# LMP88959/Digital-Subband-Video-1

Hardware: AMD Instinct MI355X
Metric: encoded Mpixels/sec, 1080p 4:2:0 GOP=12, bit-exact .dsv (higher is better)
Workload: dtype u8/int16+int32 (bit-exact; packed int16 inside a proven range, int32 escape)

## Files before the change

digital-subband-video-1_amd/csrc/k_sbt.hip:

```cpp
#include <type_traits>
#include "dsvg_dev.hpp"
#include <algorithm>
#include "dsvg_kernels.hpp"
#include "dsvg_host.hpp"

template <int M>
static __device__ __forceinline__ void store_row(int32_t *p, const int (&v)[M], int n)
{
    if (n >= M) {
        if (M == 4 && (((uintptr_t)p) & 15) == 0) {
            *reinterpret_cast<int4 *>(p) = make_int4(v[0], v[1 % M], v[2 % M], v[3 % M]);
            return;
        }
        if (M == 2 && (((uintptr_t)p) & 7) == 0) {
            *reinterpret_cast<int2 *>(p) = make_int2(v[0], v[1 % M]);
            return;
        }
#pragma unroll
        for (int i = 0; i < M; i++) p[i] = v[i];
    } else {
#pragma unroll
        for (int i = 0; i < M; i++)
            if (i < n) p[i] = v[i];
    }
// ... 358 lines not shown
static __device__ __forceinline__ s16x2 pk_rdiv2(s16x2 v) { return (v + (short)1 + (v >> 15)) >> 1; }
static __device__ __forceinline__ s16x2 pk_rdiv4(s16x2 v) { return (v + (short)2 + (v >> 15)) >> 2; }
static __device__ __forceinline__ s16x2 pk_div4(s16x2 v) { return (v + ((v >> 15) & (short)3)) >> 2; }
struct PkRow { s16x2 e0, e1, o0, o1; };
static __device__ __forceinline__ s16x2 pk_u(unsigned v) { return __builtin_bit_cast(s16x2, v); }
static __device__ __forceinline__ unsigned pk_b(s16x2 v) { return __builtin_bit_cast(unsigned, v); }
#define PK_EVEN(hi_, lo_) pk_u((lo_) & 0x00ff00ffu)
#define PK_ODD(hi_, lo_) pk_u(__builtin_amdgcn_perm(0u, (lo_), 0x0c030c01u))
#define PK_E2(hi_, lo_) pk_u(__builtin_amdgcn_perm((hi_), (lo_), 0x0c040c02u))
#define PK_O2(hi_, lo_) pk_u(__builtin_amdgcn_perm((hi_), (lo_), 0x0c050c03u))
static __device__ __forceinline__ PkRow pk_unpack8(unsigned lo, unsigned hi)
{
    return PkRow{PK_EVEN(0u, lo), PK_EVEN(0u, hi), PK_ODD(0u, lo), PK_ODD(0u, hi)};
}
static __device__ __forceinline__ void pk_bytes8(const PkRow &p, unsigned &lo, unsigned &hi)
{
    lo = (pk_b(p.o0) << 8) | pk_b(p.e0);
    hi = (pk_b(p.o1) << 8) | pk_b(p.e1);
}
template <typename EMITPK>
static __device__ __forceinline__ void mc_luma_patch_hpk(const DSVG_GLOBAL uint8_t *gr, int stride, bool xh, EMITPK emit_pk)
{
    const unsigned shb = (unsigned)(((uintptr_t)gr) & 3);
    const DSVG_GLOBAL uint8_t *ga = gr - shb;
    U4A4 rw[8];
#pragma unroll
    for (int r = 0; r < 8; r++) { const dsvg_u32x4a4 t = *reinterpret_cast<const DSVG_GLOBAL dsvg_u32x4a4 *>(ga + (r + 1) * stride); rw[r] = U4A4{t.x, t.y, t.z, t.w}; }
    __builtin_amdgcn_sched_barrier(0);
    const s16x2 z = s16x2{0, 0}, m255 = s16x2{255, 255};
    auto H = [&](s16x2 a, s16x2 b, s16x2 c, s16x2 d) {
        const s16x2 t = ((b + c) * (short)9 + (short)8 - (a + d)) >> 4;
        const s16x2 u = pk_min(pk_max(t, z), m255);
        return xh ? u : b;
    };
#pragma unroll
    for (int r = 0; r < 8; r++) {
        const unsigned lo = __builtin_amdgcn_alignbyte(rw[r].y, rw[r].x, shb), mi = __builtin_amdgcn_alignbyte(rw[r].z, rw[r].y, shb),
                       hi = __builtin_amdgcn_alignbyte(rw[r].w, rw[r].z, shb);
        const s16x2 A0 = PK_EVEN(0u, lo), A1 = PK_ODD(0u, lo), A2 = PK_E2(mi, lo), A3 = PK_O2(mi, lo), A4 = PK_EVEN(0u, mi), A5 = PK_ODD(0u, mi),
                    A6 = PK_E2(hi, mi), A7 = PK_O2(hi, mi), A8 = PK_EVEN(0u, hi);
        emit_pk(r, PkRow{H(A0, A1, A2, A3), H(A4, A5, A6, A7), H(A1, A2, A3, A4), H(A5, A6, A7, A8)});
    }
}

#define MCB(lo, mi, hi, m) ((int)((((m) < 4 ? (lo) : ((m) < 8 ? (mi) : (hi))) >> (8 * ((m) & 3))) & 0xff))
static __device__ __forceinline__ void mc_pack8(const int (&pv)[8], unsigned &plo, unsigned &phi)
{
    plo = (unsigned)pv[0] | ((unsigned)pv[1] << 8) | ((unsigned)pv[2] << 16) | ((unsigned)pv[3] << 24);
    phi = (unsigned)pv[4] | ((unsigned)pv[5] << 8) | ((unsigned)pv[6] << 16) | ((unsigned)pv[7] << 24);
}
struct NoEmitInts {};
template <bool AX, bool AY, typename EMIT, typename EMITI = NoEmitInts>
static __device__ __forceinline__ void mc_luma_patch(const DSVG_GLOBAL uint8_t *gr, int stride, bool xh, bool yh, EMIT emit, EMITI emit_i = EMITI{})
{
    auto out8 = [&](int r, const int (&pv)[8]) {
        if constexpr (std::is_same_v<EMITI, NoEmitInts>) {
            unsigned pl, ph_;
            mc_pack8(pv, pl, ph_);
            emit(r, pl, ph_);
        } else {
            emit_i(r, pv);
        }
    };
    const unsigned shb = (unsigned)(((uintptr_t)gr) & 3);
    const DSVG_GLOBAL uint8_t *ga = gr - shb;
    if (!AY) {
        U4A4 rw[8];
#pragma unroll
        for (int r = 0; r < 8; r++) { const dsvg_u32x4a4 t = *reinterpret_cast<const DSVG_GLOBAL dsvg_u32x4a4 *>(ga + (r + 1) * stride); rw[r] = U4A4{t.x, t.y, t.z, t.w}; }
        __builtin_amdgcn_sched_barrier(0);
#pragma unroll
        for (int r = 0; r < 8; r++) {
            const unsigned lo = __builtin_amdgcn_alignbyte(rw[r].y, rw[r].x, shb), mi = __builtin_amdgcn_alignbyte(rw[r].z, rw[r].y, shb),
                           hi = __builtin_amdgcn_alignbyte(rw[r].w, rw[r].z, shb);
            if (!AX) {
                emit(r, __builtin_amdgcn_alignbyte(mi, lo, 1u), __builtin_amdgcn_alignbyte(hi, mi, 1u));
            } else {
                int bq[11], pv[8];
#pragma unroll
                for (int m = 0; m < 11; m++) bq[m] = MCB(lo, mi, hi, m);
#pragma unroll
                for (int i = 0; i < 8; i++) {
                    const int t = (9 * (bq[i + 1] + bq[i + 2]) - (bq[i] + bq[i + 3]) + 8) >> 4;
                    pv[i] = xh ? d_sat8(t) : bq[i + 1];
                }
                out8(r, pv);
            }
        }
    } else {
        U4A4 rw[11];
#pragma unroll
        for (int k = 0; k < 11; k++) { const dsvg_u32x4a4 t = *reinterpret_cast<const DSVG_GLOBAL dsvg_u32x4a4 *>(ga + k * stride); rw[k] = U4A4{t.x, t.y, t.z, t.w}; }
        __builtin_amdgcn_sched_barrier(0);
        int Hq[4][8];
#pragma unroll
        for (int k = 0; k < 11; k++) {
            const unsigned lo = __builtin_amdgcn_alignbyte(rw[k].y, rw[k].x, shb), mi = __builtin_amdgcn_alignbyte(rw[k].z, rw[k].y, shb),
                           hi = __builtin_amdgcn_alignbyte(rw[k].w, rw[k].z, shb);
            int bq[11];
#pragma unroll
            for (int m = 0; m < 11; m++) bq[m] = MCB(lo, mi, hi, m);
#pragma unroll
            for (int i = 0; i < 8; i++) Hq[k & 3][i] = (AX && xh) ? 9 * (bq[i + 1] + bq[i + 2]) - (bq[i] + bq[i + 3]) : 16 * bq[i + 1];
            if (k >= 3) {
                const int r = k - 3;
                int pv[8];
#pragma unroll
                for (int i = 0; i < 8; i++) {
                    const int h0 = Hq[r & 3][i], h1 = Hq[(r + 1) & 3][i], h2 = Hq[(r + 2) & 3][i], h3 = Hq[(r + 3) & 3][i];
                    const int v = yh ? 9 * (h1 + h2) - (h0 + h3) : 16 * h1;
                    pv[i] = d_sat8((v + 128) >> 8);
                }
                out8(r, pv);
            }
        }
    }
}
template <bool AX, typename EMITPK>
static __device__ __forceinline__ void mc_luma_patch_vpk(const DSVG_GLOBAL uint8_t *gr, int stride, bool xh, bool yh, EMITPK emit_pk)
{
    const unsigned shb = (unsigned)(((uintptr_t)gr) & 3);
    const DSVG_GLOBAL uint8_t *ga = gr - shb;
    U4A4 rw[11];
#pragma unroll
    for (int k = 0; k < 11; k++) { const dsvg_u32x4a4 t = *reinterpret_cast<const DSVG_GLOBAL dsvg_u32x4a4 *>(ga + k * stride); rw[k] = U4A4{t.x, t.y, t.z, t.w}; }
    __builtin_amdgcn_sched_barrier(0);
    auto Hrow = [&](s16x2 a, s16x2 b, s16x2 c, s16x2 d) {
        const s16x2 g = b << 4;
        if (!AX) return g;
        const s16x2 f = (b + c) * (short)9 - (a + d);
        return xh ? f : g;
    };
    auto V = [&](s16x2 a0, s16x2 a1, s16x2 a2, s16x2 a3) {
        const s16x2 u = a1 + (yh ? a2 : a1), w = (yh ? a0 : a1) + (yh ? a3 : a1);
        const int vx = (9 * (int)u.x - (int)w.x + 128) >> 8, vy = (9 * (int)u.y - (int)w.y + 128) >> 8;
        return pk2(d_sat8(vx), d_sat8(vy));
    };
    PkRow Hq[4];
#pragma unroll
    for (int k = 0; k < 11; k++) {
        const unsigned lo = __builtin_amdgcn_alignbyte(rw[k].y, rw[k].x, shb), mi = __builtin_amdgcn_alignbyte(rw[k].z, rw[k].y, shb),
                       hi = __builtin_amdgcn_alignbyte(rw[k].w, rw[k].z, shb);
        const s16x2 A0 = PK_EVEN(0u, lo), A1 = PK_ODD(0u, lo), A2 = PK_E2(mi, lo), A3 = PK_O2(mi, lo), A4 = PK_EVEN(0u, mi), A5 = PK_ODD(0u, mi),
                    A6 = PK_E2(hi, mi), A7 = PK_O2(hi, mi), A8 = PK_EVEN(0u, hi);
        Hq[k & 3] = PkRow{Hrow(A0, A1, A2, A3), Hrow(A4, A5, A6, A7), Hrow(A1, A2, A3, A4), Hrow(A5, A6, A7, A8)};
        if (k >= 3) {
            const int r = k - 3;
            const PkRow &h0 = Hq[r & 3], &h1 = Hq[(r + 1) & 3], &h2 = Hq[(r + 2) & 3], &h3 = Hq[(r + 3) & 3];
            emit_pk(r, PkRow{V(h0.e0, h1.e0, h2.e0, h3.e0), V(h0.e1, h1.e1, h2.e1, h3.e1), V(h0.o0, h1.o0, h2.o0, h3.o0), V(h0.o1, h1.o1, h2.o1, h3.o1)});
        }
    }
}
struct __attribute__((aligned(4))) U3A4 { unsigned x, y, z; };
template <bool ANY, typename EMIT>
static __device__ __forceinline__ void mc_chroma_patch(const DSVG_GLOBAL uint8_t *gr, int stride, bool xh, bool yh, EMIT emit)
{
    const DSVG_GLOBAL uint8_t *g1 = gr + 1;
    const unsigned shb = (unsigned)(((uintptr_t)g1) & 3);
    const DSVG_GLOBAL uint8_t *ga = g1 - shb;
    constexpr int NR = ANY ? 9 : 8;
    U3A4 rw[NR];
#pragma unroll
    for (int k = 0; k < NR; k++) { const dsvg_u32x3a4 t = *reinterpret_cast<const DSVG_GLOBAL dsvg_u32x3a4 *>(ga + (k + 1) * stride); rw[k] = U3A4{t.x, t.y, t.z}; }
    __builtin_amdgcn_sched_barrier(0);
    unsigned qlo = 0, qhi = 0, qx = 0;
#pragma unroll
    for (int k = 0; k < NR; k++) {
        const unsigned lo = __builtin_amdgcn_alignbyte(rw[k].y, rw[k].x, shb), hi = __builtin_amdgcn_alignbyte(rw[k].z, rw[k].y, shb),
                       x8 = rw[k].z >> (8 * shb);
        if (!ANY) {
            emit(k, lo, hi);
        } else if (k >= 1) {
            int pv[8];
#pragma unroll
            for (int i = 0; i < 8; i++) {
                const int pa = MCB(qlo, qhi, qx, i), pb = MCB(qlo, qhi, qx, i + 1), pc = MCB(lo, hi, x8, i), pd = MCB(lo, hi, x8, i + 1);
                const int B = xh ? pb : pa, C = yh ? pc : pa, D = xh ? (yh ? pd : pb) : (yh ? pc : pa);
                pv[i] = (pa + B + C + D + 2) >> 2;
            }
            unsigned pl, ph_;
            mc_pack8(pv, pl, ph_);
            emit(k - 1, pl, ph_);
        }
        qlo = lo; qhi = hi; qx = x8;
    }
}

template <typename EMITPK>
static __device__ __forceinline__ void mc_chroma_patch_pk(const DSVG_GLOBAL uint8_t *gr, int stride, bool xh, bool yh, EMITPK emit_pk)
{
    const DSVG_GLOBAL uint8_t *g1 = gr + 1;
    const unsigned shb = (unsigned)(((uintptr_t)g1) & 3);
    const DSVG_GLOBAL uint8_t *ga = g1 - shb;
    U3A4 rw[9];
#pragma unroll
    for (int k = 0; k < 9; k++) { const dsvg_u32x3a4 t = *reinterpret_cast<const DSVG_GLOBAL dsvg_u32x3a4 *>(ga + (k + 1) * stride); rw[k] = U3A4{t.x, t.y, t.z}; }
    __builtin_amdgcn_sched_barrier(0);
    const s16x2 two = s16x2{2, 2};
    PkRow hp;
#pragma unroll
    for (int k = 0; k < 9; k++) {
        const unsigned lo = __builtin_amdgcn_alignbyte(rw[k].y, rw[k].x, shb), hi = __builtin_amdgcn_alignbyte(rw[k].z, rw[k].y, shb),
                       x8 = rw[k].z >> (8 * shb);
        const s16x2 A0 = PK_EVEN(0u, lo), A1 = PK_ODD(0u, lo), A2 = PK_E2(hi, lo), A4 = PK_EVEN(0u, hi), A5 = PK_ODD(0u, hi), A6 = PK_E2(x8, hi);
        const PkRow h = PkRow{A0 + (xh ? A1 : A0), A4 + (xh ? A5 : A4), A1 + (xh ? A2 : A1), A5 + (xh ? A6 : A5)};
        if (k >= 1)
            emit_pk(k - 1, PkRow{(hp.e0 + (yh ? h.e0 : hp.e0) + two) >> 2, (hp.e1 + (yh ? h.e1 : hp.e1) + two) >> 2,
                                 (hp.o0 + (yh ? h.o0 : hp.o0) + two) >> 2, (hp.o1 + (yh ? h.o1 : hp.o1) + two) >> 2});
        hp = h;
    }
}

struct FwdFastQ {
    int sh1[4];
    int q2[2], q3;
    float rc2[2], rc3;
};
static __device__ __forceinline__ int sym_shift(int v, int sh) { return (v + ((v >> 31) & ((1 << sh) - 1))) >> sh; }
static __device__ __forceinline__ void put_row4(const QCtx &q, int pos, s16x2 ab, s16x2 cd)
{
    const unsigned x = __builtin_bit_cast(unsigned, ab), y = __builtin_bit_cast(unsigned, cd);
    if (!(x | y)) return;
#ifndef FWD_FAST_NO_ROW4
    if ((pos & 3) == 0) {
        typedef unsigned row4_t __attribute__((ext_vector_type(2)));
        row4_t v;
        v.x = x; v.y = y;
        *reinterpret_cast<DSVG_GLOBAL row4_t *>(q.sym + pos) = v;
        q.nzf[pos >> 2] = 1;
        q.cfl[pos >> 11] = 1;
        return;
    }
#endif
    if (ab.x) q.put_sparse(pos, ab.x);
    if (ab.y) q.put_sparse(pos + 1, ab.y);
    if (cd.x) q.put_sparse(pos + 2, cd.x);
    if (cd.y) q.put_sparse(pos + 3, cd.y);
}
static __device__ __forceinline__ void put_row4(const QCtx &q, int pos, int a, int b, int c, int d)
{
    if (!(a | b | c | d)) return;
#ifndef FWD_FAST_NO_ROW4
    if ((pos & 3) == 0) {
        typedef unsigned row4_t __attribute__((ext_vector_type(2)));
        row4_t v;
        v.x = ((unsigned)a & 0xffffu) | ((unsigned)b << 16);
        v.y = ((unsigned)c & 0xffffu) | ((unsigned)d << 16);
        *reinterpret_cast<DSVG_GLOBAL row4_t *>(q.sym + pos) = v;
        q.nzf[pos >> 2] = 1;
        q.cfl[pos >> 11] = 1;
        return;
    }
#endif
    if (a) q.put_sparse(pos, a);
    if (b) q.put_sparse(pos + 1, b);
    if (c) q.put_sparse(pos + 2, c);
    if (d) q.put_sparse(pos + 3, d);
}

static __device__ __forceinline__ void fwd_fast_rows1(const QCtx &q, const QLevel &L1, int sh1, int cx1, int cy1,
                                                      const int (&r0)[8], const int (&r1)[8], int (&out)[4])
{
    int mx = max(r0[0], r0[1]), mn = min(r0[0], r0[1]);
#pragma unroll
    for (int i = 2; i < 8; i += 2) { mx = max(mx, max(r0[i], r0[i + 1])); mn = min(mn, min(r0[i], r0[i + 1])); }
#pragma unroll
    for (int i = 0; i < 8; i += 2) { mx = max(mx, max(r1[i], r1[i + 1])); mn = min(mn, min(r1[i], r1[i + 1])); }
    if (4 * max(mx, -mn) < (1 << sh1)) {
#pragma unroll
        for (int i = 0; i < 4; i++) out[i] = (r0[2 * i] + r0[2 * i + 1]) + (r1[2 * i] + r1[2 * i + 1]);
        return;
    }
    int slh[4], shl[4], shh[4], any = 0;
#pragma unroll
    for (int i = 0; i < 4; i++) {
        const int s0 = r0[2 * i] + r0[2 * i + 1], s1 = r1[2 * i] + r1[2 * i + 1];
        const int d0 = r0[2 * i] - r0[2 * i + 1], d1 = r1[2 * i] - r1[2 * i + 1];
        out[i] = s0 + s1;
        slh[i] = sym_shift(d0 + d1, sh1); shl[i] = sym_shift(s0 - s1, sh1); shh[i] = sym_shift(d0 - d1, sh1);
        any |= slh[i] | shl[i] | shh[i];
    }
    if (any) {
        q.nz_any = 1;
        const int pr = cy1 * L1.sw + cx1;
        put_row4(q, L1.base0 + pr, slh[0], slh[1], slh[2], slh[3]);
        put_row4(q, L1.base1 + pr, shl[0], shl[1], shl[2], shl[3]);
        put_row4(q, L1.base2 + pr, shh[0], shh[1], shh[2], shh[3]);
    }
}
static __device__ __forceinline__ void fwd_fast_rows1_pk(const QCtx &q, const QLevel &L1, int sh1, int cx1, int cy1,
                                                         const PkRow &r0, const PkRow &r1, int (&out)[4])
{
    const s16x2 s0a = r0.e0 + r0.o0, s0b = r0.e1 + r0.o1, d0a = r0.e0 - r0.o0, d0b = r0.e1 - r0.o1;
    const s16x2 s1a = r1.e0 + r1.o0, s1b = r1.e1 + r1.o1, d1a = r1.e0 - r1.o0, d1b = r1.e1 - r1.o1;
    const s16x2 lla = s0a + s1a, llb = s0b + s1b;
    const s16x2 lha = d0a + d1a, lhb = d0b + d1b, hla = s0a - s1a, hlb = s0b - s1b, hha = d0a - d1a, hhb = d0b - d1b;
    out[0] = lla.x; out[1] = lla.y; out[2] = llb.x; out[3] = llb.y;
    const s16x2 mx = pk_max(pk_max(pk_max(lha, lhb), pk_max(hla, hlb)), pk_max(hha, hhb));
    const s16x2 mn = pk_min(pk_min(pk_min(lha, lhb), pk_min(hla, hlb)), pk_min(hha, hhb));
    const s16x2 am = pk_max(mx, s16x2{0, 0} - mn);
    if ((pk_b(am) & ~(((1u << min(sh1, 15)) - 1u) * 0x00010001u)) == 0) return;
    q.nz_any = 1;
    const int pr = cy1 * L1.sw + cx1;
    const short ms = (short)((1 << sh1) - 1), ss = (short)sh1;
    const s16x2 mm = {ms, ms}, sv = {ss, ss}, s15 = {15, 15};
    auto pks = [&](s16x2 v) { return (v + ((v >> s15) & mm)) >> sv; };
    put_row4(q, L1.base0 + pr, pks(lha), pks(lhb));
    put_row4(q, L1.base1 + pr, pks(hla), pks(hlb));
    put_row4(q, L1.base2 + pr, pks(hha), pks(hhb));
}
template <int N, int HZL>
static __device__ __forceinline__ void fwd_fast_level(const QCtx &q, const QLevel &L, const int (&qqv)[N / 2], const float (&rcv)[N / 2], int cx0, int cy0,
                                                      const int (&in)[N][N], int (&out)[N / 2][N / 2])
{
#pragma unroll
    for (int j = 0; j < N / 2; j++)
#pragma unroll
        for (int i = 0; i < N / 2; i++) {
            const int qq = qqv[j];
            const float rc = rcv[j];
            const int a = in[2 * j][2 * i], b = in[2 * j][2 * i + 1], c = in[2 * j + 1][2 * i], d = in[2 * j + 1][2 * i + 1];
            const int s0 = a + b, s1 = c + d, d0 = a - b, d1 = c - d;
            out[j][i] = d_ll_down(s0 + s1);
            const int vlh = d0 + d1, vhl = s0 - s1, vhh = d0 - d1;
#ifndef FWD_FAST_NO_QTEST
            if (max(max(max(vlh, vhl), vhh), -min(min(vlh, vhl), vhh)) < qq) continue;
#endif
            int slh, shl, shh;
            (void)q_coef<HZL>(qq, rc, vlh, slh);
            (void)q_coef<HZL>(qq, rc, vhl, shl);
            (void)q_coef<HZL>(qq, rc, vhh, shh);
            if (slh | shl | shh) {
                q.nz_any = 1;
                const int pr = (cy0 + j) * L.sw + cx0 + i;
                if (slh) q.put_sparse(L.base0 + pr, slh);
                if (shl) q.put_sparse(L.base1 + pr, shl);
                if (shh) q.put_sparse(L.base2 + pr, shh);
            }
        }
}

#ifndef FWD_FAST_INTRA
#define FWD_FAST_INTRA 1
#endif
struct FwdFastSel { bool ok, intra; QLevel L1, L2, L3; int i1[4], i2[2], i3; };
struct FwdFastHp { QLevel L1, L2, L3; int nbh; bool ovx, ovy, sparse; };
static __device__ __forceinline__ FwdFastHp fwd_fast_hp(const JobDev &jb, const HzPlane &hp)
{
    FwdFastHp H;
    const int sw0 = hp.s_w[0], sw1 = hp.s_w[1], sw2 = hp.s_w[2], sh0 = hp.s_h[0], sh1 = hp.s_h[1], sh2 = hp.s_h[2];
    H.L1 = q_level<2>(hp); H.L2 = q_level<1>(hp); H.L3 = q_level<0>(hp);
    H.nbh = hp.nbh;
    H.ovx = (int)(2 * sw0 > sw1) | (int)(2 * sw1 > sw2);
    H.ovy = (int)(2 * sh0 > sh1) | (int)(2 * sh1 > sh2);
    H.sparse = jb.nzf != nullptr;
    return H;
}
static __device__ __forceinline__ FwdFastSel fwd_fast_sel(const FwdFastHp &H, int mode, int I, int J, int x0, int y0, int pw, int ph)
{
    FwdFastSel S;
    S.ok = false; S.intra = mode != 0;
    if (H.sparse && (FWD_FAST_INTRA || mode == 0) && x0 + 8 <= pw && y0 + 8 <= ph && !(H.ovx && I == 0) && !(H.ovy && J == 0)) {
        S.L1 = H.L1; S.L2 = H.L2; S.L3 = H.L3;
        const int nbh = H.nbh;
        const int b1x = (4 * I * S.L1.dbx) >> 14, b2x = (2 * I * S.L2.dbx) >> 14;
        S.ok = b1x == ((4 * I + 3) * S.L1.dbx) >> 14 && b2x == ((2 * I + 1) * S.L2.dbx) >> 14;
#pragma unroll
        for (int j = 0; j < 4; j++) S.i1[j] = (((4 * J + j) * S.L1.dby) >> 14) * nbh + b1x;
#pragma unroll
        for (int j = 0; j < 2; j++) S.i2[j] = (((2 * J + j) * S.L2.dby) >> 14) * nbh + b2x;
        S.i3 = ((J * S.L3.dby) >> 14) * nbh + ((I * S.L3.dbx) >> 14);
    }
    return S;
}
static __device__ __forceinline__ FwdFastSel fwd_fast_sel(const JobDev &jb, const HzPlane &hp, bool any_ov, int mode, int I, int J,
                                                          int x0, int y0, int pw, int ph)
{
    (void)any_ov;
    return fwd_fast_sel(fwd_fast_hp(jb, hp), mode, I, J, x0, y0, pw, ph);
}

template <int CH>
static __device__ __forceinline__ void fwd_mc_fast_body(const JobDev *__restrict__ jobs, const SbtGeo3 &G, const McGeo &MG, int c0, int npl,
                                                        const DMV *__restrict__ mvs0, XcdGrid XG, int plain)
{
    Blk3 B;
    if (!d_xcd_blk3(XG, B, plain != 0)) return;
    int job, c;
    d_job_plane(B.z, npl, c0, job, c);
    const SbtGeo g = G.g[c];
    const int I = B.x * 64 + threadIdx.x, J = B.y * 4 + threadIdx.y;
    if (I >= g.w3 || J >= g.h3) return;
    const JobDev &jb = jobs[job];
    const int sh = CH ? MG.hs : 0, sv = CH ? MG.vs : 0;
    const int bw = MG.blk_w >> sh, bh = MG.blk_h >> sv;
    const int pw = MG.w[c], ph = g.ph, stride = g.pstride;
    const int x0 = 8 * I, y0 = 8 * J;
    const int bi = (int)(((float)I + 0.5f) * __builtin_amdgcn_rcpf((float)(bw >> 3)));
    const int bj = (int)(((float)J + 0.5f) * __builtin_amdgcn_rcpf((float)(bh >> 3)));
    const int nblk = MG.nbh * MG.nbv, blk = bj * MG.nbh + bi;
    const HzPlane &hp = jb.hz[c];
    FwdFastHp H = fwd_fast_hp(jb, hp);
    const DMV *mvtab = jb.mvs;
    const uint8_t *stable_p = jb.stable, *srcp_p = jb.srcp[c];
    int sstride = jb.srcs[c];
#define FWD_PIN(x) asm volatile("" : "+s"(x))
#ifndef FWD_FAST_NO_PIN
    FWD_PIN(H.L1.sh0); FWD_PIN(H.L1.sh1); FWD_PIN(H.L1.dbx); FWD_PIN(H.L1.dby); FWD_PIN(H.L2.qp); FWD_PIN(H.L2.dbx); FWD_PIN(H.L2.dby);
    FWD_PIN(H.L3.qp); FWD_PIN(H.L3.dbx); FWD_PIN(H.L3.dby); FWD_PIN(H.nbh); FWD_PIN(mvtab); FWD_PIN(stable_p); FWD_PIN(srcp_p); FWD_PIN(sstride);
#endif
    DMV mv;
    {
        const auto mq = reinterpret_cast<const DSVG_GLOBAL char *>(dsvg_global(mvs0 ? mvs0 + (size_t)job * nblk : mvtab)) + (unsigned)blk * (unsigned)sizeof(DMV);
        const unsigned xy = *reinterpret_cast<const DSVG_GLOBAL unsigned *>(mq);
        mv.x = (int16_t)(xy & 0xffffu); mv.y = (int16_t)(xy >> 16); mv.mode = *reinterpret_cast<const DSVG_GLOBAL uint8_t *>(mq + 4);
    }
    QCtx q;
    q.hp = &hp; q.stable = dsvg_global(stable_p);
    q.sym = dsvg_global(jb.sym + jb.nz_off[c]);
    q.any_ov = H.ovx | H.ovy;
    q.nzf = H.sparse ? dsvg_global(jb.nzf + (jb.nz_off[c] >> 2)) : nullptr;
    q.cfl = H.sparse ? dsvg_global(jb.cflag + jb.chunk_off[c]) : nullptr;
    const FwdFastSel S = fwd_fast_sel(H, mv.mode, I, J, x0, y0, pw, ph);
    if (!S.ok) return;
    const QLevel &L1 = S.L1, &L2 = S.L2, &L3 = S.L3;
    const auto sp = dsvg_global(srcp_p);
    uint2 sw[8];
    if (S.intra) {
        const auto px = dsvg_global(static_cast<const uint8_t *>(jb.xf + g.poff));
#pragma unroll
        for (int r = 0; r < 8; r++) sw[r] = dsvg_ld2(px + (unsigned)((y0 + r) * stride + x0));
    } else {
#pragma unroll
        for (int r = 0; r < 8; r++) sw[r] = dsvg_ld2(sp + (unsigned)((y0 + r) * sstride + x0));
    }
    int f1[4], f2[2];
#pragma unroll
    for (int j = 0; j < 4; j++) f1[j] = q.stable[S.i1[j]];
#pragma unroll
    for (int j = 0; j < 2; j++) f2[j] = q.stable[S.i2[j]];
    const int f3 = q.stable[S.i3];
    FwdFastQ fq;
    const int dx = mv.x >> sh, dy = mv.y >> sv;
    const int xb = bi * bw, yb = bj * bh;
    const int wx = d_clamp(xb + (dx >> 1), -DSVG_BORDER, pw - bw + DSVG_BORDER - 1) + (x0 - xb);
    const int wy = d_clamp(yb + (dy >> 1), -DSVG_BORDER, ph - bh + DSVG_BORDER - 1) + (y0 - yb);
    const bool xh = !S.intra && (dx & 1), yh = !S.intra && (dy & 1);
    const auto gr = dsvg_global(static_cast<const uint8_t *>(jb.ref + g.poff)) + ((wy - 1) * stride + (wx - 1));
    const bool any_x = __ballot(xh) != 0ull, any_y = __ballot(yh) != 0ull;
    const auto pp = dsvg_global(jb.pred + g.poff);
#ifndef FWD_FAST_NO_PK
    int l1[4][4];
    PkRow rp[2];
    const s16x2 cmin = s16x2{-128, -128}, cmax = s16x2{127, 127};
    auto emit_core = [&](int r, const PkRow &P, unsigned plo, unsigned phi) {
        const PkRow Sr = pk_unpack8(sw[r].x, sw[r].y);
        PkRow &R = rp[r & 1];
        R.e0 = pk_min(pk_max(Sr.e0 - P.e0, cmin), cmax); R.e1 = pk_min(pk_max(Sr.e1 - P.e1, cmin), cmax);
        R.o0 = pk_min(pk_max(Sr.o0 - P.o0, cmin), cmax); R.o1 = pk_min(pk_max(Sr.o1 - P.o1, cmin), cmax);
        dsvg_st2(pp + (unsigned)((y0 + r) * stride + x0), make_uint2(plo, phi));
        if (r & 1) fwd_fast_rows1_pk(q, L1, f1[r >> 1] ? L1.sh1 : L1.sh0, 4 * I, 4 * J + (r >> 1), rp[0], rp[1], l1[r >> 1]);
    };
    auto emit = [&](int r, unsigned plo, unsigned phi) { emit_core(r, pk_unpack8(plo, phi), plo, phi); };
    auto emit_pk = [&](int r, const PkRow &P) {
        unsigned plo, phi;
        pk_bytes8(P, plo, phi);
        emit_core(r, P, plo, phi);
    };
    if (S.intra) {
        const s16x2 c128 = s16x2{128, 128};
#pragma unroll
        for (int r = 0; r < 8; r++) {
            const PkRow X = pk_unpack8(sw[r].x, sw[r].y);
            PkRow &R = rp[r & 1];
            R.e0 = X.e0 - c128; R.e1 = X.e1 - c128; R.o0 = X.o0 - c128; R.o1 = X.o1 - c128;
            if (r & 1) fwd_fast_rows1_pk(q, L1, f1[r >> 1] ? L1.sh1 : L1.sh0, 4 * I, 4 * J + (r >> 1), rp[0], rp[1], l1[r >> 1]);
        }
    } else
#ifdef FWD_FAST_NO_VPK
    auto emit_i = [&](int r, const int (&pv)[8]) { emit_pk(r, PkRow{pk2(pv[0], pv[2]), pk2(pv[4], pv[6]), pk2(pv[1], pv[3]), pk2(pv[5], pv[7])}); };
#endif
    if (CH == 0) {
#ifdef FWD_FAST_NO_VPK
        if (any_y) mc_luma_patch<true, true>(gr, stride, xh, yh, emit, emit_i);
#else
        if (any_y && any_x) mc_luma_patch_vpk<true>(gr, stride, xh, yh, emit_pk);
        else if (any_y) mc_luma_patch_vpk<false>(gr, stride, xh, yh, emit_pk);
#endif
        else if (any_x) mc_luma_patch_hpk(gr, stride, xh, emit_pk);
        else mc_luma_patch<false, false>(gr, stride, xh, yh, emit);
    } else {
        if (any_x || any_y) mc_chroma_patch_pk(gr, stride, xh, yh, emit_pk);
        else mc_chroma_patch<false>(gr, stride, xh, yh, emit);
    }
#else
    int l1[4][4], ra[2][8];
    auto emit = [&](int r, unsigned plo, unsigned phi) {
        int (&row)[8] = ra[r & 1];
#pragma unroll
        for (int i = 0; i < 8; i++) {
            const int sv_ = (int)(((i < 4 ? sw[r].x : sw[r].y) >> (8 * (i & 3))) & 0xff);
            const int pv_ = (int)(((i < 4 ? plo : phi) >> (8 * (i & 3))) & 0xff);
            row[i] = d_clamp(sv_ - pv_, -128, 127);
        }
        dsvg_st2(pp + (unsigned)((y0 + r) * stride + x0), make_uint2(plo, phi));
        if (r & 1) fwd_fast_rows1(q, L1, f1[r >> 1] ? L1.sh1 : L1.sh0, 4 * I, 4 * J + (r >> 1), ra[0], ra[1], l1[r >> 1]);
    };
    if (CH == 0) {
        if (any_y) mc_luma_patch<true, true>(gr, stride, xh, yh, emit);
        else if (any_x) mc_luma_patch<true, false>(gr, stride, xh, yh, emit);
        else mc_luma_patch<false, false>(gr, stride, xh, yh, emit);
    } else {
        if (any_x || any_y) mc_chroma_patch<true>(gr, stride, xh, yh, emit);
        else mc_chroma_patch<false>(gr, stride, xh, yh, emit);
    }
#endif
#pragma unroll
    for (int j = 0; j < 2; j++) {
        fq.q2[j] = max(L2.qp >> ((f2[j] & 2) ? 2 : (f2[j] != 0)), HZ_MINQ);
        fq.rc2[j] = __builtin_amdgcn_rcpf((float)(fq.q2[j] << 1));
    }
    fq.q3 = max(L3.qp >> ((f3 & 2) ? 2 : (f3 != 0)), HZ_MINQ);
    fq.rc3 = __builtin_amdgcn_rcpf((float)(fq.q3 << 1));
    int l2[2][2], l3[1][1];
    fwd_fast_level<4, 1>(q, L2, fq.q2, fq.rc2, 2 * I, 2 * J, l1, l2);
    const int q3v[1] = {fq.q3};
    const float rc3v[1] = {fq.rc3};
    fwd_fast_level<2, 0>(q, L3, q3v, rc3v, I, J, l2, l3);
    dsvg_global(jb.s3 + g.s3off)[(unsigned)(J * g.w3 + I)] = l3[0][0];
    dsvg_global(jb.pflag + g.s3off)[(unsigned)(J * g.w3 + I)] = (uint8_t)q.nz_any;
}
#ifndef FAST_WPE_L
#define FAST_WPE_L 4
#endif
#ifndef FAST_WPE_C
#define FAST_WPE_C 0
#endif
#if FAST_WPE_L > 0
#define FAST_WPE_L_ATTR __attribute__((amdgpu_waves_per_eu(FAST_WPE_L, FAST_WPE_L)))
#else
#define FAST_WPE_L_ATTR
#endif
#if FAST_WPE_C > 0
#define FAST_WPE_C_ATTR __attribute__((amdgpu_waves_per_eu(FAST_WPE_C, FAST_WPE_C)))
#else
#define FAST_WPE_C_ATTR
#endif
template <int CH>
__global__ void k_fwd_mc_fast(const JobDev *__restrict__ jobs, SbtGeo3 G, McGeo MG, int c0, int npl, const DMV *__restrict__ mvs0, XcdGrid XG, int plain);
template <>
__global__ __launch_bounds__(256) FAST_WPE_L_ATTR void k_fwd_mc_fast<0>(const JobDev *__restrict__ jobs, SbtGeo3 G, McGeo MG, int c0, int npl,
                                                                        const DMV *__restrict__ mvs0, XcdGrid XG, int plain)
{
    DSVG_CLK_BEGIN();
    fwd_mc_fast_body<0>(jobs, G, MG, c0, npl, mvs0, XG, plain);
    DSVG_CLK_END(1);
}
template <>
__global__ __launch_bounds__(256) FAST_WPE_C_ATTR void k_fwd_mc_fast<1>(const JobDev *__restrict__ jobs, SbtGeo3 G, McGeo MG, int c0, int npl,
                                                                        const DMV *__restrict__ mvs0, XcdGrid XG, int plain)
{
    DSVG_CLK_BEGIN();
    fwd_mc_fast_body<1>(jobs, G, MG, c0, npl, mvs0, XG, plain);
    DSVG_CLK_END(2);
}

template <int CH>
__global__ __launch_bounds__(256) void k_mc_patch(const JobDev *__restrict__ jobs, SbtGeo3 G, McGeo MG, int c0, int npl, const DMV *__restrict__ mvs0,
                                                  XcdGrid XG, int ex0, int ey0)
{
    Blk3 B;
    if (!d_xcd_blk3(XG, B)) return;
    int job, c;
    d_job_plane(B.z, npl, c0, job, c);
    const SbtGeo g = G.g[c];
    const int I = B.x * 64 + threadIdx.x, J = B.y * 4 + threadIdx.y;
    if (I >= g.w3 || J >= g.h3) return;
    const JobDev &jb = jobs[job];
    const int sh = CH ? MG.hs : 0, sv = CH ? MG.vs : 0;
    const int bw = MG.blk_w >> sh, bh = MG.blk_h >> sv;
    const int pw = MG.w[c], ph = g.ph, stride = g.pstride;
    const int x0 = 8 * I, y0 = 8 * J;
    if (x0 + 8 > pw || y0 + 8 > ph) return;
    const int bi = (int)(((float)I + 0.5f) * __builtin_amdgcn_rcpf((float)(bw >> 3)));
    const int bj = (int)(((float)J + 0.5f) * __builtin_amdgcn_rcpf((float)(bh >> 3)));
    if (bi >= ex0 || bj >= ey0) return;
    const int nblk = MG.nbh * MG.nbv, blk = bj * MG.nbh + bi;
    const DMV mv = mvs0 ? mvs0[(size_t)job * nblk + blk] : jb.mvs[blk];
    if (mv.mode != 0) return;
    const int dx = mv.x >> sh, dy = mv.y >> sv;
    const int xb = bi * bw, yb = bj * bh;
    const int wx = d_clamp(xb + (dx >> 1), -DSVG_BORDER, pw - bw + DSVG_BORDER - 1) + (x0 - xb);
    const int wy = d_clamp(yb + (dy >> 1), -DSVG_BORDER, ph - bh + DSVG_BORDER - 1) + (y0 - yb);
    const bool xh = dx & 1, yh = dy & 1;
    const auto gr = dsvg_global(static_cast<const uint8_t *>(jb.ref + g.poff)) + ((wy - 1) * stride + (wx - 1));
    const bool any_x = __ballot(xh) != 0ull, any_y = __ballot(yh) != 0ull;
    const auto pp = dsvg_global(jb.pred + g.poff);
    auto emit = [&](int r, unsigned plo, unsigned phi) { dsvg_st2(pp + (unsigned)((y0 + r) * stride + x0), make_uint2(plo, phi)); };
    auto emit_pk = [&](int r, const PkRow &P) {
        unsigned plo, phi;
        pk_bytes8(P, plo, phi);
        dsvg_st2(pp + (unsigned)((y0 + r) * stride + x0), make_uint2(plo, phi));
    };
    if (CH == 0) {
        if (any_y && any_x) mc_luma_patch_vpk<true>(gr, stride, xh, yh, emit_pk);
        else if (any_y) mc_luma_patch_vpk<false>(gr, stride, xh, yh, emit_pk);
        else if (any_x) mc_luma_patch_hpk(gr, stride, xh, emit_pk);
        else mc_luma_patch<false, false>(gr, stride, xh, yh, emit);
    } else {
        if (any_x || any_y) mc_chroma_patch_pk(gr, stride, xh, yh, emit_pk);
        else mc_chroma_patch<false>(gr, stride, xh, yh, emit);
    }
}

#ifndef MC_WPE
#define MC_WPE 4
#endif
#if MC_WPE > 0
#define MC_WPE_ATTR __attribute__((amdgpu_waves_per_eu(MC_WPE)))
#else
#define MC_WPE_ATTR
#endif
template <int CH>
__global__ __launch_bounds__(256) MC_WPE_ATTR void k_fwd_mc_pix(const JobDev *__restrict__ jobs, SbtGeo3 G, McGeo MG, int c0, int npl,
                                                    const DMV *__restrict__ mvs0, int skip_fast, int bxofs, int byofs, int bxstep, int bystep)
{
    int job, c;
    d_job_plane((int)blockIdx.z, npl, c0, job, c);
    const SbtGeo g = G.g[c];
    const int I = (bxofs + (int)blockIdx.x * bxstep) * 64 + threadIdx.x, J = (byofs + (int)blockIdx.y * bystep) * 4 + threadIdx.y;
    if (I >= g.w3 || J >= g.h3) return;
    const JobDev &jb = jobs[job];
    const int sh = CH ? MG.hs : 0, sv = CH ? MG.vs : 0;
    const int bw = MG.blk_w >> sh, bh = MG.blk_h >> sv;
    const int pw = MG.w[c], ph = g.ph, stride = g.pstride;
    const int x0 = 8 * I, y0 = 8 * J;
    const int bi = (int)(((float)I + 0.5f) * __builtin_amdgcn_rcpf((float)(bw >> 3)));
    const int bj = (int)(((float)J + 0.5f) * __builtin_amdgcn_rcpf((float)(bh >> 3)));
    const int nblk = MG.nbh * MG.nbv, blk = bj * MG.nbh + bi;
    const DMV mv = mvs0 ? mvs0[(size_t)job * nblk + blk] : jb.mvs[blk];
    int32_t *coef = jb.coef + g.coff;
    const int W = g.W, H = g.H;
    const int wo1 = DSVG_RSU(W, 1), ho1 = DSVG_RSU(H, 1), wo2 = DSVG_RSU(W, 2), ho2 = DSVG_RSU(H, 2);
    QCtx q;
    const HzPlane &hp = jb.hz[c];
    q.hp = &hp; q.stable = dsvg_global(jb.stable);
    q.sym = dsvg_global(jb.sym + jb.nz_off[c]);
    q.any_ov = (2 * hp.s_w[0] > hp.s_w[1]) || (2 * hp.s_h[0] > hp.s_h[1]) ||
               (2 * hp.s_w[1] > hp.s_w[2]) || (2 * hp.s_h[1] > hp.s_h[2]);
    q.nzf = jb.nzf ? dsvg_global(jb.nzf + (jb.nz_off[c] >> 2)) : nullptr;
    q.cfl = jb.nzf ? dsvg_global(jb.cflag + jb.chunk_off[c]) : nullptr;
    if (skip_fast && fwd_fast_sel(jb, hp, q.any_ov, mv.mode, I, J, x0, y0, pw, ph).ok) return;
#ifdef AB_COUNT_GENERAL
    if (jb.stat) atomicAdd(jb.stat + 64 * (2 + (c != 0)) + (threadIdx.x & 63), 1u);
#endif
    HaarQ<8, 2> hq1;
    hq1.init(q, 4 * I, 4 * J, W, H, wo1, ho1);
    int l1[4][4], ra[2][8];

    if (mv.mode != 0) {
        const auto px = dsvg_global(static_cast<const uint8_t *>(jb.xf + g.poff));
#pragma unroll
        for (int r = 0; r < 8; r++) {
            const int y = y0 + r;
            uint2 v = make_uint2(0x80808080u, 0x80808080u);
            if (y < ph) v = dsvg_ld2(px + (unsigned)(y * stride + x0));
#pragma unroll
            for (int i = 0; i < 4; i++) {
                ra[r & 1][i] = (int)((v.x >> (8 * i)) & 0xff) - 128;
                ra[r & 1][i + 4] = (int)((v.y >> (8 * i)) & 0xff) - 128;
            }
            if (r & 1) hq1.rows(q, r >> 1, ra[0], ra[1], l1[r >> 1], false);
        }
    } else {
        const auto sp = dsvg_global(jb.srcp[c]);
        const int sstride = jb.srcs[c];
        uint2 sw[8];
#pragma unroll
        for (int r = 0; r < 8; r++) sw[r] = dsvg_ld2(sp + (unsigned)(min(y0 + r, ph - 1) * sstride + x0));
        const int dx = mv.x >> sh, dy = mv.y >> sv;
        const int xb = bi * bw, yb = bj * bh;
        const int wx = d_clamp(xb + (dx >> 1), -DSVG_BORDER, pw - bw + DSVG_BORDER - 1) + (x0 - xb);
        const int wy = d_clamp(yb + (dy >> 1), -DSVG_BORDER, ph - bh + DSVG_BORDER - 1) + (y0 - yb);
        const bool xh = dx & 1, yh = dy & 1;
        const auto gr = dsvg_global(static_cast<const uint8_t *>(jb.ref + g.poff)) + ((wy - 1) * stride + (wx - 1));
        const bool any_x = __ballot(xh) != 0ull, any_y = __ballot(yh) != 0ull;
        const auto pp = dsvg_global(jb.pred + g.poff);
        const bool inside = x0 + 8 <= pw && y0 + 8 <= ph;
        auto emit = [&](int r, unsigned plo, unsigned phi) {
            int (&row)[8] = ra[r & 1];
#pragma unroll
            for (int i = 0; i < 8; i++) {
                const int sv_ = (int)(((i < 4 ? sw[r].x : sw[r].y) >> (8 * (i & 3))) & 0xff);
                const int pv_ = (int)(((i < 4 ? plo : phi) >> (8 * (i & 3))) & 0xff);
                row[i] = d_clamp(sv_ - pv_, -128, 127);
            }
            if (inside) {
                dsvg_st2(pp + (unsigned)((y0 + r) * stride + x0), make_uint2(plo, phi));
            } else {
                const int y = y0 + r;
#pragma unroll
                for (int i = 0; i < 8; i++) {
                    if (y >= ph) row[i] = 0;
                    else if (x0 + i < pw) pp[(size_t)y * stride + x0 + i] = (uint8_t)((i < 4 ? plo : phi) >> (8 * (i & 3)));
                    else {
                        const int e = (int)(((i - 1 < 4 ? sw[r].x : sw[r].y) >> (8 * ((i - 1) & 3))) & 0xff);
                        row[i] = (x0 + i == pw && MG.cw_extra[c] && i > 0) ? e - 128 : 0;
                    }
                }
            }
            if (r & 1) hq1.rows(q, r >> 1, ra[0], ra[1], l1[r >> 1], false);
        };
        if (CH == 0) {
            if (any_y) mc_luma_patch<true, true>(gr, stride, xh, yh, emit);
            else if (any_x) mc_luma_patch<true, false>(gr, stride, xh, yh, emit);
            else mc_luma_patch<false, false>(gr, stride, xh, yh, emit);
        } else {
            if (any_x || any_y) mc_chroma_patch<true>(gr, stride, xh, yh, emit);
            else mc_chroma_patch<false>(gr, stride, xh, yh, emit);
        }
    }
    int l2[2][2], l3[1][1];
    haar_fwd_patch_q<4, 1>(l1, l2, 2 * I, 2 * J, wo1, ho1, W, wo2, ho2, coef, true, q);
    haar_fwd_patch_q<2, 0>(l2, l3, I, J, wo2, ho2, W, g.w3, g.h3, coef, true, q);
    dsvg_global(jb.s3 + g.s3off)[(unsigned)(J * g.w3 + I)] = l3[0][0];
    if (jb.nzf) dsvg_global(jb.pflag + g.s3off)[(unsigned)(J * g.w3 + I)] = (uint8_t)q.nz_any;
}

#ifndef FWD_B4T_WPE
#define FWD_B4T_WPE 6
#endif
#if FWD_B4T_WPE
#define FWD_B4T_ATTR __attribute__((amdgpu_waves_per_eu(FWD_B4T_WPE, FWD_B4T_WPE)))
#else
#define FWD_B4T_ATTR
#endif
template <bool Q>
__global__ __launch_bounds__(256) FWD_B4T_ATTR void k_fwd_b4t(const JobDev *__restrict__ jobs, SbtGeo3 G, int c0, int npl,
                                                 int from_src)
{
    int job, c;
    d_job_plane((int)blockIdx.z, npl, c0, job, c);
    const SbtGeo g = G.g[c];
    const int W = g.W, H = g.H;
    const int I = blockIdx.x * 64 + threadIdx.x, J = blockIdx.y * 4 + threadIdx.y;
    if (8 * I >= W || 8 * J >= H) return;
    const JobDev &jb = jobs[job];
    const uint8_t *px = from_src ? jb.srcp[c] : jb.xf + g.poff;
    const int pxs = from_src ? jb.srcs[c] : g.pstride;
    int32_t *coef = jb.coef + g.coff;
    const int hw = W >> 1, hh = H >> 1;

    int RL[4][4], RH[4][4];
    const int nC = min(4, max(0, hw - 4 * I));
    QCtx q;
    QLevel Lq;
    int cls[4][4];
    bool chx = false, chy = false;
    if (Q) {
        const HzPlane &hp = jb.hz[c];
        q.hp = &hp; q.stable = dsvg_global(jb.stable);
        q.sym = dsvg_global(jb.sym + jb.nz_off[c]);
        q.any_ov = (2 * hp.s_w[0] > hp.s_w[1]) || (2 * hp.s_h[0] > hp.s_h[1]) ||
                   (2 * hp.s_w[1] > hp.s_w[2]) || (2 * hp.s_h[1] > hp.s_h[2]);
        Lq = q_level<2>(hp);
        q_flags<2, 4>(q, Lq, 4 * I, 4 * J, hw, hh, cls);
        chx = q.any_ov && I == 0; chy = q.any_ov && J == 0;
    }
#ifndef FWD_B4T_NO_PK
    if constexpr (Q) {
        if (W - 1 - 8 * I >= 7) {
            const bool ledge = I == 0, redge = 8 * I + 8 > W - 1;
            const auto pxg = dsvg_global(px);
            s16x2 RL[4][2], RH[4][2];
            s16x2 shv[4][2];
#pragma unroll
            for (int m = 0; m < 4; m++)
#pragma unroll
                for (int h = 0; h < 2; h++)
                    shv[m][h] = s16x2{(short)min(cls[m][2 * h] ? Lq.sh1 : Lq.sh0, 15), (short)min(cls[m][2 * h + 1] ? Lq.sh1 : Lq.sh0, 15)};
            const s16x2 c512 = s16x2{512, 512};
#ifndef FB4T_AHEAD
#define FB4T_AHEAD 3
#endif
            uint2 mmv[10];
            unsigned lfv[10], rgv[10];
            auto request = [&](int r) {
                int y = 8 * J - 1 + r;
                y = y < 0 ? 1 : (y > H - 1 ? H - 1 : y);
                const unsigned ro = (unsigned)(min(y, g.ph - 1) * pxs + 8 * I);
                mmv[r] = dsvg_ld2(pxg + ro);
                lfv[r] = *reinterpret_cast<const DSVG_GLOBAL unsigned *>(pxg + (ledge ? ro : ro - 4u));
                rgv[r] = *reinterpret_cast<const DSVG_GLOBAL unsigned *>(pxg + (redge ? ro + 4u : ro + 8u));
            };
#pragma unroll
            for (int r = 0; r < FB4T_AHEAD && r < 10; r++) request(r);
#pragma unroll
            for (int r = 0; r < 10; r++) {
                int y = 8 * J - 1 + r;
                y = y < 0 ? 1 : (y > H - 1 ? H - 1 : y);
                if (r + FB4T_AHEAD < 10) request(r + FB4T_AHEAD);
                unsigned lo, mi, hi;
                {
                    const uint2 mm = mmv[r];
                    const unsigned lft = lfv[r], rgt = rgv[r];
// ... 1988 lines not shown
```

Before: 248,600.

## Extend chroma fast MC path to cover top and bottom edge tile rows

Adds an EDGE specialization of the fused forward MC/transform fast path for chroma. It takes tiles at the bottom edge where only 4 rows remain, and top-row tiles with vertical overlap, which previously fell back to the slower general kernel. Edge handling clamps row loads, zeroes missing rows, duplicates level-2 rows, and chains the top-row HL coefficient. The chroma kernel picks the edge variant per wave through readfirstlane, and the general kernel skips tiles the fast path now covers. This adds code size and bit-exactness risk at the plane edges.

Result: slower. 238,900 (-3.9%).

```diff
diff --git a/digital-subband-video-1_amd/csrc/k_sbt.hip b/digital-subband-video-1_amd/csrc/k_sbt.hip
--- a/digital-subband-video-1_amd/csrc/k_sbt.hip
+++ b/digital-subband-video-1_amd/csrc/k_sbt.hip
@@ -534,8 +534,8 @@
     }
 }
 struct __attribute__((aligned(4))) U3A4 { unsigned x, y, z; };
-template <bool ANY, typename EMIT>
-static __device__ __forceinline__ void mc_chroma_patch(const DSVG_GLOBAL uint8_t *gr, int stride, bool xh, bool yh, EMIT emit)
+template <bool ANY, bool LIM = false, typename EMIT>
+static __device__ __forceinline__ void mc_chroma_patch(const DSVG_GLOBAL uint8_t *gr, int stride, bool xh, bool yh, EMIT emit, int nr = 8)
 {
     const DSVG_GLOBAL uint8_t *g1 = gr + 1;
     const unsigned shb = (unsigned)(((uintptr_t)g1) & 3);
@@ -543,7 +543,7 @@
     constexpr int NR = ANY ? 9 : 8;
     U3A4 rw[NR];
 #pragma unroll
-    for (int k = 0; k < NR; k++) { const dsvg_u32x3a4 t = *reinterpret_cast<const DSVG_GLOBAL dsvg_u32x3a4 *>(ga + (k + 1) * stride); rw[k] = U3A4{t.x, t.y, t.z}; }
+    for (int k = 0; k < NR; k++) { const dsvg_u32x3a4 t = *reinterpret_cast<const DSVG_GLOBAL dsvg_u32x3a4 *>(ga + ((LIM ? min(k, nr - (ANY ? 0 : 1)) : k) + 1) * stride); rw[k] = U3A4{t.x, t.y, t.z}; }
     __builtin_amdgcn_sched_barrier(0);
     unsigned qlo = 0, qhi = 0, qx = 0;
 #pragma unroll
@@ -568,15 +568,15 @@
     }
 }
 
-template <typename EMITPK>
-static __device__ __forceinline__ void mc_chroma_patch_pk(const DSVG_GLOBAL uint8_t *gr, int stride, bool xh, bool yh, EMITPK emit_pk)
+template <bool LIM = false, typename EMITPK>
+static __device__ __forceinline__ void mc_chroma_patch_pk(const DSVG_GLOBAL uint8_t *gr, int stride, bool xh, bool yh, EMITPK emit_pk, int nr = 8)
 {
     const DSVG_GLOBAL uint8_t *g1 = gr + 1;
     const unsigned shb = (unsigned)(((uintptr_t)g1) & 3);
     const DSVG_GLOBAL uint8_t *ga = g1 - shb;
     U3A4 rw[9];
 #pragma unroll
-    for (int k = 0; k < 9; k++) { const dsvg_u32x3a4 t = *reinterpret_cast<const DSVG_GLOBAL dsvg_u32x3a4 *>(ga + (k + 1) * stride); rw[k] = U3A4{t.x, t.y, t.z}; }
+    for (int k = 0; k < 9; k++) { const dsvg_u32x3a4 t = *reinterpret_cast<const DSVG_GLOBAL dsvg_u32x3a4 *>(ga + ((LIM ? min(k, nr) : k) + 1) * stride); rw[k] = U3A4{t.x, t.y, t.z}; }
     __builtin_amdgcn_sched_barrier(0);
     const s16x2 two = s16x2{2, 2};
     PkRow hp;
@@ -691,9 +691,9 @@
     put_row4(q, L1.base1 + pr, pks(hla), pks(hlb));
     put_row4(q, L1.base2 + pr, pks(hha), pks(hhb));
 }
-template <int N, int HZL>
+template <int N, int HZL, bool CHAIN = false>
 static __device__ __forceinline__ void fwd_fast_level(const QCtx &q, const QLevel &L, const int (&qqv)[N / 2], const float (&rcv)[N / 2], int cx0, int cy0,
-                                                      const int (&in)[N][N], int (&out)[N / 2][N / 2])
+                                                      const int (&in)[N][N], int (&out)[N / 2][N / 2], bool chain = false, int ho = 0)
 {
 #pragma unroll
     for (int j = 0; j < N / 2; j++)
@@ -704,7 +704,9 @@
             const int a = in[2 * j][2 * i], b = in[2 * j][2 * i + 1], c = in[2 * j + 1][2 * i], d = in[2 * j + 1][2 * i + 1];
             const int s0 = a + b, s1 = c + d, d0 = a - b, d1 = c - d;
             out[j][i] = d_ll_down(s0 + s1);
-            const int vlh = d0 + d1, vhl = s0 - s1, vhh = d0 - d1;
+            const int vlh = d0 + d1, vhh = d0 - d1;
+            int vhl = s0 - s1;
+            if (CHAIN && j == 0 && chain) vhl = q_chain(q, HZL, cx0 + i, ho, vhl);
 #ifndef FWD_FAST_NO_QTEST
             if (max(max(max(vlh, vhl), vhh), -min(min(vlh, vhl), vhh)) < qq) continue;
 #endif
@@ -725,49 +727,53 @@
 #ifndef FWD_FAST_INTRA
 #define FWD_FAST_INTRA 1
 #endif
-struct FwdFastSel { bool ok, intra; QLevel L1, L2, L3; int i1[4], i2[2], i3; };
-struct FwdFastHp { QLevel L1, L2, L3; int nbh; bool ovx, ovy, sparse; };
+struct FwdFastSel { bool ok, intra, bot, top; QLevel L1, L2, L3; int i1[4], i2[2], i3; };
+struct FwdFastHp { QLevel L1, L2, L3; int nbh, sh1; bool ovx, ovy, ovy3, sparse; };
 static __device__ __forceinline__ FwdFastHp fwd_fast_hp(const JobDev &jb, const HzPlane &hp)
 {
     FwdFastHp H;
     const int sw0 = hp.s_w[0], sw1 = hp.s_w[1], sw2 = hp.s_w[2], sh0 = hp.s_h[0], sh1 = hp.s_h[1], sh2 = hp.s_h[2];
     H.L1 = q_level<2>(hp); H.L2 = q_level<1>(hp); H.L3 = q_level<0>(hp);
-    H.nbh = hp.nbh;
+    H.nbh = hp.nbh; H.sh1 = sh1;
     H.ovx = (int)(2 * sw0 > sw1) | (int)(2 * sw1 > sw2);
     H.ovy = (int)(2 * sh0 > sh1) | (int)(2 * sh1 > sh2);
+    H.ovy3 = 2 * sh0 > sh1 && !(2 * sh1 > sh2);
     H.sparse = jb.nzf != nullptr;
     return H;
 }
+template <bool EDGE = false>
 static __device__ __forceinline__ FwdFastSel fwd_fast_sel(const FwdFastHp &H, int mode, int I, int J, int x0, int y0, int pw, int ph)
 {
     FwdFastSel S;
     S.ok = false; S.intra = mode != 0;
-    if (H.sparse && (FWD_FAST_INTRA || mode == 0) && x0 + 8 <= pw && y0 + 8 <= ph && !(H.ovx && I == 0) && !(H.ovy && J == 0)) {
+    const bool shy = H.ovy && J == 0, full = y0 + 8 <= ph;
+    S.bot = EDGE && y0 + 4 == ph && mode == 0 && !shy;
+    S.top = EDGE && shy && H.ovy3 && mode == 0 && full;
+    if (H.sparse && (FWD_FAST_INTRA || mode == 0) && x0 + 8 <= pw && (full || S.bot) && !(H.ovx && I == 0) && (!shy || S.top)) {
         S.L1 = H.L1; S.L2 = H.L2; S.L3 = H.L3;
         const int nbh = H.nbh;
         const int b1x = (4 * I * S.L1.dbx) >> 14, b2x = (2 * I * S.L2.dbx) >> 14;
         S.ok = b1x == ((4 * I + 3) * S.L1.dbx) >> 14 && b2x == ((2 * I + 1) * S.L2.dbx) >> 14;
 #pragma unroll
-        for (int j = 0; j < 4; j++) S.i1[j] = (((4 * J + j) * S.L1.dby) >> 14) * nbh + b1x;
-#pragma unroll
-        for (int j = 0; j < 2; j++) S.i2[j] = (((2 * J + j) * S.L2.dby) >> 14) * nbh + b2x;
+        for (int j = 0; j < 4; j++) S.i1[j] = (((4 * J + (S.bot && j > 1 ? 1 : j)) * S.L1.dby) >> 14) * nbh + b1x;
+#pragma unroll
+        for (int j = 0; j < 2; j++) S.i2[j] = (((2 * J + (S.bot ? 0 : j)) * S.L2.dby) >> 14) * nbh + b2x;
         S.i3 = ((J * S.L3.dby) >> 14) * nbh + ((I * S.L3.dbx) >> 14);
     }
     return S;
 }
+template <bool EDGE>
 static __device__ __forceinline__ FwdFastSel fwd_fast_sel(const JobDev &jb, const HzPlane &hp, bool any_ov, int mode, int I, int J,
                                                           int x0, int y0, int pw, int ph)
 {
     (void)any_ov;
-    return fwd_fast_sel(fwd_fast_hp(jb, hp), mode, I, J, x0, y0, pw, ph);
-}
-
-template <int CH>
+    return fwd_fast_sel<EDGE>(fwd_fast_hp(jb, hp), mode, I, J, x0, y0, pw, ph);
+}
+
+template <int CH, bool EDGE>
 static __device__ __forceinline__ void fwd_mc_fast_body(const JobDev *__restrict__ jobs, const SbtGeo3 &G, const McGeo &MG, int c0, int npl,
-                                                        const DMV *__restrict__ mvs0, XcdGrid XG, int plain)
-{
-    Blk3 B;
-    if (!d_xcd_blk3(XG, B, plain != 0)) return;
+                                                        const DMV *__restrict__ mvs0, const Blk3 &B)
+{
     int job, c;
     d_job_plane(B.z, npl, c0, job, c);
     const SbtGeo g = G.g[c];
@@ -803,7 +809,7 @@
     q.any_ov = H.ovx | H.ovy;
     q.nzf = H.sparse ? dsvg_global(jb.nzf + (jb.nz_off[c] >> 2)) : nullptr;
     q.cfl = H.sparse ? dsvg_global(jb.cflag + jb.chunk_off[c]) : nullptr;
-    const FwdFastSel S = fwd_fast_sel(H, mv.mode, I, J, x0, y0, pw, ph);
+    const FwdFastSel S = fwd_fast_sel<EDGE>(H, mv.mode, I, J, x0, y0, pw, ph);
     if (!S.ok) return;
     const QLevel &L1 = S.L1, &L2 = S.L2, &L3 = S.L3;
     const auto sp = dsvg_global(srcp_p);
@@ -814,7 +820,7 @@
         for (int r = 0; r < 8; r++) sw[r] = dsvg_ld2(px + (unsigned)((y0 + r) * stride + x0));
     } else {
 #pragma unroll
-        for (int r = 0; r < 8; r++) sw[r] = dsvg_ld2(sp + (unsigned)((y0 + r) * sstride + x0));
+        for (int r = 0; r < 8; r++) sw[r] = dsvg_ld2(sp + (unsigned)((EDGE ? min(y0 + r, ph - 1) : y0 + r) * sstride + x0));
     }
     int f1[4], f2[2];
 #pragma unroll
@@ -836,6 +842,10 @@
     PkRow rp[2];
     const s16x2 cmin = s16x2{-128, -128}, cmax = s16x2{127, 127};
     auto emit_core = [&](int r, const PkRow &P, unsigned plo, unsigned phi) {
+        if (EDGE && r >= 4 && S.bot) {
+            if (r & 1) { l1[r >> 1][0] = 0; l1[r >> 1][1] = 0; l1[r >> 1][2] = 0; l1[r >> 1][3] = 0; }
+            return;
+        }
         const PkRow Sr = pk_unpack8(sw[r].x, sw[r].y);
         PkRow &R = rp[r & 1];
         R.e0 = pk_min(pk_max(Sr.e0 - P.e0, cmin), cmax); R.e1 = pk_min(pk_max(Sr.e1 - P.e1, cmin), cmax);
@@ -872,10 +882,12 @@
         else if (any_x) mc_luma_patch_hpk(gr, stride, xh, emit_pk);
         else mc_luma_patch<false, false>(gr, stride, xh, yh, emit);
     } else {
-        if (any_x || any_y) mc_chroma_patch_pk(gr, stride, xh, yh, emit_pk);
-        else mc_chroma_patch<false>(gr, stride, xh, yh, emit);
+        const int nr = EDGE && S.bot ? 4 : 8;
+        if (any_x || any_y) mc_chroma_patch_pk<EDGE>(gr, stride, xh, yh, emit_pk, nr);
+        else mc_chroma_patch<false, EDGE>(gr, stride, xh, yh, emit, nr);
     }
 #else
+    static_assert(!EDGE, "the edge rows exist in the packed build only");
     int l1[4][4], ra[2][8];
     auto emit = [&](int r, unsigned plo, unsigned phi) {
         int (&row)[8] = ra[r & 1];
@@ -905,7 +917,8 @@
     fq.q3 = max(L3.qp >> ((f3 & 2) ? 2 : (f3 != 0)), HZ_MINQ);
     fq.rc3 = __builtin_amdgcn_rcpf((float)(fq.q3 << 1));
     int l2[2][2], l3[1][1];
-    fwd_fast_level<4, 1>(q, L2, fq.q2, fq.rc2, 2 * I, 2 * J, l1, l2);
+    fwd_fast_level<4, 1, EDGE>(q, L2, fq.q2, fq.rc2, 2 * I, 2 * J, l1, l2, EDGE && S.top, H.sh1);
+    if (EDGE && S.bot) { l2[1][0] = l2[0][0]; l2[1][1] = l2[0][1]; }
     const int q3v[1] = {fq.q3};
     const float rc3v[1] = {fq.rc3};
     fwd_fast_level<2, 0>(q, L3, q3v, rc3v, I, J, l2, l3);
@@ -935,7 +948,8 @@
                                                                         const DMV *__restrict__ mvs0, XcdGrid XG, int plain)
 {
     DSVG_CLK_BEGIN();
-    fwd_mc_fast_body<0>(jobs, G, MG, c0, npl, mvs0, XG, plain);
+    Blk3 B;
+    if (d_xcd_blk3(XG, B, plain != 0)) fwd_mc_fast_body<0, false>(jobs, G, MG, c0, npl, mvs0, B);
     DSVG_CLK_END(1);
 }
 template <>
@@ -943,7 +957,14 @@
                                                                         const DMV *__restrict__ mvs0, XcdGrid XG, int plain)
 {
     DSVG_CLK_BEGIN();
-    fwd_mc_fast_body<1>(jobs, G, MG, c0, npl, mvs0, XG, plain);
+    Blk3 B;
+    if (d_xcd_blk3(XG, B, plain != 0)) {
+        int job, c;
+        d_job_plane(B.z, npl, c0, job, c);
+        const int J = B.y * 4 + (int)threadIdx.y;
+        if (__builtin_amdgcn_readfirstlane((int)(J == 0 || J == G.g[c].h3 - 1))) fwd_mc_fast_body<1, true>(jobs, G, MG, c0, npl, mvs0, B);
+        else fwd_mc_fast_body<1, false>(jobs, G, MG, c0, npl, mvs0, B);
+    }
     DSVG_CLK_END(2);
 }
 
@@ -1032,7 +1053,7 @@
                (2 * hp.s_w[1] > hp.s_w[2]) || (2 * hp.s_h[1] > hp.s_h[2]);
     q.nzf = jb.nzf ? dsvg_global(jb.nzf + (jb.nz_off[c] >> 2)) : nullptr;
     q.cfl = jb.nzf ? dsvg_global(jb.cflag + jb.chunk_off[c]) : nullptr;
-    if (skip_fast && fwd_fast_sel(jb, hp, q.any_ov, mv.mode, I, J, x0, y0, pw, ph).ok) return;
+    if (skip_fast && fwd_fast_sel<CH != 0>(jb, hp, q.any_ov, mv.mode, I, J, x0, y0, pw, ph).ok) return;
 #ifdef AB_COUNT_GENERAL
     if (jb.stat) atomicAdd(jb.stat + 64 * (2 + (c != 0)) + (threadIdx.x & 63), 1u);
 #endif
```
